# nabeelscicom/DistilCodec_nabeel

Measured on AMD Instinct MI355X. Metric: 24 kHz samples/s encode+decode at 1/8 GPU; code-index bit-exact vs CPU, higher is better.
Workload: dtype f32

## Files before the change

distilcodec_nabeel_amd/csrc/dcx_conv_common.h:

```cpp
#pragma once
#include <algorithm>
#include <type_traits>

#include "dcx_kernels.h"
#include "dcx_planes.h"

namespace dcx {

typedef float f32x16 __attribute__((ext_vector_type(16)));
typedef float f32x4 __attribute__((ext_vector_type(4)));
typedef float f32x2 __attribute__((ext_vector_type(2)));
typedef short s16x8 __attribute__((ext_vector_type(8)));
typedef short s16x4 __attribute__((ext_vector_type(4)));
typedef __bf16 bf16x8 __attribute__((ext_vector_type(8)));

constexpr int BK = 16;
constexpr int LDSK = 20;
template <bool SWZ>
struct XRow {
  static constexpr int kStride = SWZ ? 48 : 56;
  __device__ static __forceinline__ int half(int row, int h) { return SWZ ? h ^ ((row >> 3) & 1) : h; }
  __device__ static __forceinline__ int off(int row, int piece) {
    const int h = piece >= 3;
    return row * kStride + (half(row, h) * 3 + piece - 3 * h) * 8;
  }
};

__device__ __forceinline__ float silu_f(float v) { return v * __builtin_amdgcn_rcpf(1.0f + __expf(-v)); }
__device__ __forceinline__ float gelu_f(float v) { return 0.5f * v * (1.0f + erff(v * 0.70710678118654752440f)); }
__device__ __forceinline__ float gelu_bf16_f(float v) {
#ifdef DCX_GELU_ERF
  return gelu_f(v);
#endif
  const float z = fabsf(v) * 0.70710678118654752440f;
  const float t = __builtin_amdgcn_rcpf(fmaf(0.5f, z, 1.0f));
  float q = 0.17087277f;
  q = fmaf(q, t, -0.82215223f);
  q = fmaf(q, t, 1.48851587f);
  q = fmaf(q, t, -1.13520398f);
  q = fmaf(q, t, 0.27886807f);
  q = fmaf(q, t, -0.18628806f);
  q = fmaf(q, t, 0.09678418f);
  q = fmaf(q, t, 0.37409196f);
  q = fmaf(q, t, 1.00002368f);
  const float c = t * __expf(fmaf(t, q, fmaf(-z, z, -1.26551223f)));
  const float e = v >= 0.0f ? 1.0f - c : c - 1.0f;
  return 0.5f * v * (1.0f + e);
}

__device__ __forceinline__ f32x2 gelu_bf16_f2(f32x2 v) {
#ifdef DCX_GELU_SCALAR
  return f32x2{gelu_bf16_f(v[0]), gelu_bf16_f(v[1])};
#endif
  const f32x2 z = __builtin_elementwise_abs(v) * 0.70710678118654752440f;
  const f32x2 d = __builtin_elementwise_fma(f32x2{0.5f, 0.5f}, z, f32x2{1.0f, 1.0f});
  const f32x2 t = {__builtin_amdgcn_rcpf(d[0]), __builtin_amdgcn_rcpf(d[1])};
  auto fm = [&](f32x2 q, float c) { return __builtin_elementwise_fma(q, t, f32x2{c, c}); };
  f32x2 q = {0.17087277f, 0.17087277f};
  q = fm(q, -0.82215223f);
  q = fm(q, 1.48851587f);
  q = fm(q, -1.13520398f);
  q = fm(q, 0.27886807f);
  q = fm(q, -0.18628806f);
  q = fm(q, 0.09678418f);
  q = fm(q, 0.37409196f);
  q = fm(q, 1.00002368f);
  const f32x2 arg = __builtin_elementwise_fma(t, q, __builtin_elementwise_fma(-z, z, f32x2{-1.26551223f, -1.26551223f}));
  const f32x2 c = t * f32x2{__expf(arg[0]), __expf(arg[1])};
  const f32x2 e = {v[0] >= 0.0f ? 1.0f - c[0] : c[0] - 1.0f, v[1] >= 0.0f ? 1.0f - c[1] : c[1] - 1.0f};
  return 0.5f * v * (1.0f + e);
}

__device__ __forceinline__ int xcd_remap(int bid, int nwg) {
  const int xcd = bid & 7, q = nwg >> 3, r = nwg & 7;
  return (xcd < r ? xcd * (q + 1) : r * (q + 1) + (xcd - r) * q) + (bid >> 3);
}

__device__ __forceinline__ void flat_tile(int tpc, int batch, int& wg, int& b, int& ph) {
  const int t = xcd_remap(blockIdx.x, gridDim.x);
  const int per_ph = tpc * batch;
  ph = t / per_ph;
  const int r = t - ph * per_ph;
  b = r / tpc;
  wg = r - b * tpc;
}

__device__ __forceinline__ void ksplit_slice(const ConvParams& p, int b, int& clip, int& c0, int& nchunks) {
  clip = b;
  c0 = 0;
  nchunks = p.Cin / BK;
  if (p.ksplit > 1) {
    const int clips = p.batch / p.ksplit, sl = b / clips;
    clip = b - sl * clips;
    const int nunits = nchunks / p.kunit, base = nunits / p.ksplit, extra = nunits % p.ksplit;
    c0 = (sl * base + min(sl, extra)) * p.kunit;
    nchunks = (base + (sl < extra ? 1 : 0)) * p.kunit;
  }
}

static __device__ __attribute__((used, aligned(16))) float g_zero_row[32] = {0.f};

#if defined(DCX_CLOCK_DIAG) || defined(DCX_SEG_DIAG) || defined(DCX_TILE_DIAG)
#define DCX_DIAG 1
constexpr int kTileDiagMax = 16384;
[[maybe_unused]] static __device__ unsigned long long g_clock_diag[3], g_seg_diag[13], g_seg_diag8[49];
[[maybe_unused]] static __device__ unsigned long long g_tile_diag[kTileDiagMax * 6];
[[maybe_unused]] static __device__ unsigned int g_tile_cnt;
enum DiagSet : int { DIAG_CLOCK, DIAG_SEG, DIAG_SEG8, DIAG_TILES };
static int diag_read(int set, unsigned long long* out, int n, int reset) {
  if (set == DIAG_TILES) {
    unsigned int cnt = 0;
    if (hipMemcpyFromSymbol(&cnt, HIP_SYMBOL(g_tile_cnt), sizeof cnt) != hipSuccess) return -1;
    cnt = std::min(cnt, (unsigned)std::max(0, std::min(n, kTileDiagMax)));
    if (cnt && hipMemcpyFromSymbol(out, HIP_SYMBOL(g_tile_diag), sizeof(unsigned long long) * 6 * cnt) != hipSuccess) return -1;
    const unsigned int z = 0;
    if (reset && hipMemcpyToSymbol(HIP_SYMBOL(g_tile_cnt), &z, sizeof z) != hipSuccess) return -1;
    return (int)cnt;
  }
  const void* sym = set == DIAG_CLOCK ? (const void*)g_clock_diag : set == DIAG_SEG ? (const void*)g_seg_diag : (const void*)g_seg_diag8;
  unsigned long long v[49] = {};
  if (n > 49 || hipMemcpyFromSymbol(v, sym, sizeof(unsigned long long) * n) != hipSuccess) return -1;
  for (int i = 0; i < n; ++i) out[i] += v[i];
  const unsigned long long z[49] = {};
  if (reset && hipMemcpyToSymbol(sym, z, sizeof(unsigned long long) * n) != hipSuccess) return -1;
  return 0;
}
#define DCX_DIAG_FILE(tag) \
  int diag_##tag(int set, unsigned long long* out, int n, int reset) { return diag_read(set, out, n, reset); }
#else
#define DCX_DIAG_FILE(tag)
#endif
#ifdef DCX_SEG_DIAG
#define DCX_SEGT(v) const unsigned long long v = __builtin_amdgcn_s_memtime()
#else
#define DCX_SEGT(v)
#endif
#ifdef DCX_TILE_DIAG
#define DCX_TILET(v) const unsigned long long v = __builtin_amdgcn_s_memrealtime()
#else
#define DCX_TILET(v)
#endif

struct EpiPre {
  int osh;
  float acur;
  bool track;
};
template <int RROW>
__device__ __forceinline__ EpiPre epi_range_pre(const ConvParams& p, const ConvParams& pr, int b) {
  EpiPre e{0, 0.f, false};
  const bool h2o = (p.y6 && p.y_layout == LAYOUT_H2) || (p.y6s && p.ys_layout != LAYOUT_PLANES);
  const bool h2row = (RROW & 2) && h2o && pr.yb.rowwise;
  if (h2o && !h2row) {
    const float bnd = range_bound(pr.yb, b);
    e.osh = __builtin_amdgcn_readfirstlane(h2_shift(bnd));
    if (threadIdx.x == 0) {
      if (pr.y_ash) pr.y_ash[b] = e.osh;
      if (pr.rflag && !(bnd <= 3.0e38f)) atomicOr(pr.rflag, RANGE_NONFINITE);
    }
  }
  const bool track = pr.y_amax != nullptr;
  e.track = track;
  e.acur = track && !h2row ? __builtin_bit_cast(float, __builtin_amdgcn_readfirstlane(
                                                           __builtin_bit_cast(int, range_cur(pr.y_amax, b))))
                           : 0.f;
  return e;
}

struct EpiGeneric {
  static constexpr bool fixed = false;
};
template <int EPI, int MEAN, bool Y, bool Y2, bool Y6H, bool Y6SH, bool TRACK, bool ROWWISE = false>
struct EpiForm {
  static constexpr bool fixed = true;
  static constexpr int epi = EPI, mean = MEAN;
  static constexpr bool y = Y, y2 = Y2, y6h = Y6H, y6sh = Y6SH, track = TRACK, rowwise = ROWWISE;
};
template <typename F>
inline bool epi_form_is(const ConvParams& p) {
  const bool h2o = F::y6h || F::y6sh;
  return p.epi == F::epi && p.mean_mode == F::mean && !p.round_bf16 && (p.y != nullptr) == F::y &&
         (p.y2 != nullptr) == F::y2 && (p.y6 != nullptr) == F::y6h && (p.y6s != nullptr) == F::y6sh &&
         (!p.y6 || p.y_layout == LAYOUT_H2) && (!p.y6s || p.ys_layout == LAYOUT_H2) && (p.y_amax != nullptr) == F::track &&
         (h2o ? (p.yb.rowwise != 0) == F::rowwise : true) && (F::epi != EPI_GELU || p.w6 != nullptr) &&
         (F::mean == MEAN_NONE || p.macc != nullptr);
}

template <int BM, int BN, int WM, int WN, int LDS_FLOATS, int NT, int RROW, bool RAG, typename F, typename AccT>
__device__ __forceinline__ void epilogue_form(const ConvParams& p, const ConvParams& pr, AccT& acc, int q0, int co0, int b,
                                              int ph, float* smem, const EpiPre& pre) {
  constexpr int WR = BM / WM, WC = BN / WN;
  static_assert(sizeof(acc[0][0]) == 16 && sizeof(acc) == WR * WC * 4 / 64, "16 x 16 accumulator blocks");
  constexpr int LDSW = BN + 4;
  constexpr int RPP = (BM * LDSW <= LDS_FLOATS) ? BM
                      : (BM / 2 * LDSW <= LDS_FLOATS) ? BM / 2
                      : (BM / 4 * LDSW <= LDS_FLOATS) ? BM / 4 : WR;
  static_assert(RPP % WR == 0 && RPP * LDSW <= LDS_FLOATS, "epilogue pass does not fit LDS");
  const int tid = threadIdx.x, lane = tid & 63, wave = tid >> 6;
  const int wm = wave / WN, wn = wave % WN;
  const long long ob = (long long)b * p.y_bstride;
  constexpr bool RIN = RROW & 1, ROUT = RROW & 2;
  constexpr bool h2o = F::y6h || F::y6sh, h2row = ROUT && h2o && F::rowwise;
  constexpr bool need_r = F::epi == EPI_GAMMA_RES || F::epi == EPI_RES;
  constexpr bool need_m = F::mean == MEAN_MID || F::mean == MEAN_LAST;
  static_assert(!((F::mean == MEAN_FIRST || F::mean == MEAN_MID) && (F::y || F::y2 || h2o || F::track)), "mean form");
  unsigned short* const y6 = F::y6h ? p.y6 + ob * 2 : nullptr;
  unsigned short* const y6s = F::y6sh ? p.y6s + ob * 2 : nullptr;
  const float osc = __builtin_bit_cast(
      float, __builtin_amdgcn_readfirstlane(__builtin_bit_cast(int, __builtin_ldexpf(1.0f, h2o && !h2row ? pre.osh : 0))));
  float vmax = 0.f;
  const int lq_live = RAG ? clip_rows(pr.clip_len, pr.len_mul, b, p.Lq) : p.Lq;
  constexpr int G = 8, NH = 2;
  static_assert(NT % (BN / G) == 0, "each thread keeps one channel group");
  const int cg = (tid % (BN / G)) * G, trow = tid / (BN / G), co = co0 + cg;
  const int hsw = (lane >> 3) & 1;
  f32x4 bias4[NH], gamma4[NH];
#pragma unroll
  for (int h = 0; h < NH; ++h) {
    bias4[h] = p.bias ? *reinterpret_cast<const f32x4*>(p.bias + co + 4 * h) : f32x4{0.f, 0.f, 0.f, 0.f};
    gamma4[h] = F::epi == EPI_GAMMA_RES ? *reinterpret_cast<const f32x4*>(p.gamma + co + 4 * h) : f32x4{0.f, 0.f, 0.f, 0.f};
  }
  constexpr int RSTEP = NT / (BN / G), ROWS_T = RPP / RSTEP;
  static_assert(RPP % RSTEP == 0, "epilogue rows per thread");
  constexpr auto div_cap = [](int n, int cap) {
    int d = n < cap ? n : cap;
    while (n % d) --d;
    return d;
  };
  constexpr int IB = div_cap(ROWS_T, need_r || need_m ? 4 / NH : 8 / NH);
  auto row_bound = [&](int q) { return fmaf(pr.yb.g[0], fmaxf(pr.yb.m[0][(long long)b * p.Lq + q], pr.yb.f[0]), pr.yb.c); };

  auto pass = [&](int r0, auto fullt) {
    constexpr bool FULL = decltype(fullt)::value;
    f32x4 r[IB][NH], m[IB][NH];
    float rin[RIN ? IB : 1], rbnd[h2row ? IB : 1];
    auto load = [&](int rb) {
#pragma unroll
      for (int k = 0; k < IB; ++k) {
        const int qq = q0 + r0 + trow + (rb + k) * RSTEP;
        const int q = FULL ? qq : min(qq, p.Lq - 1);
        const long long o = ob + ((long long)q * p.out_mul + ph) * p.ldy + co;
#pragma unroll
        for (int h = 0; h < NH; ++h) {
          if constexpr (need_r) r[k][h] = *reinterpret_cast<const f32x4*>(p.res + o + 4 * h);
          if constexpr (need_m) m[k][h] = *reinterpret_cast<const f32x4*>(p.macc + o + 4 * h);
        }
        if constexpr (RIN) rin[k] = pr.x_ash_row ? __builtin_ldexpf(1.0f, -pr.x_ash_row[(long long)b * p.Lin + q]) : 1.0f;
        if constexpr (h2row) rbnd[k] = row_bound(q);
      }
    };
    load(0);
    __syncthreads();
    if (wm * WR >= r0 && wm * WR < r0 + RPP) {
#pragma unroll
      for (int i = 0; i < WR / 16; ++i)
#pragma unroll
        for (int j = 0; j < WC / 16; ++j)
#pragma unroll
          for (int e = 0; e < 4; ++e) {
            const int row = wm * WR + i * 16 + 4 * (lane >> 4) + e - r0;
            smem[row * LDSW + wn * WC + j * 16 + (lane & 15)] = acc[i][j][e];
          }
    }
    __syncthreads();
#pragma unroll
    for (int rb = 0; rb < ROWS_T; rb += IB) {
      f32x4 x[IB][NH];
      float rsc[IB];
#pragma unroll
      for (int k = 0; k < IB; ++k) {
        const int rl = trow + (rb + k) * RSTEP;
        const int q = q0 + r0 + rl;
        const bool dead = RAG && q >= lq_live;
        const float rin_ = RIN ? rin[RIN ? k : 0] : 1.0f;
        const f32x4 u = *reinterpret_cast<const f32x4*>(smem + rl * LDSW + cg + 4 * hsw);
        const f32x4 v = *reinterpret_cast<const f32x4*>(smem + rl * LDSW + cg + 4 * (1 - hsw));
        x[k][0] = (hsw ? v : u) * rin_ + bias4[0];
        x[k][1] = (hsw ? u : v) * rin_ + bias4[1];
#pragma unroll
        for (int h = 0; h < NH; ++h) {
          if constexpr (F::epi == EPI_GELU) {
#pragma unroll
            for (int e = 0; e < 4; e += 2) {
              const f32x2 g = gelu_bf16_f2(f32x2{x[k][h][e], x[k][h][e + 1]});
              x[k][h][e] = g[0];
              x[k][h][e + 1] = g[1];
            }
          } else if constexpr (F::epi == EPI_GAMMA_RES) {
            x[k][h] = r[k][h] + gamma4[h] * x[k][h];
          } else if constexpr (F::epi == EPI_RES) {
            x[k][h] = r[k][h] + x[k][h];
          } else {
            static_assert(F::epi == EPI_BIAS, "epilogue form");
          }
          if (dead) x[k][h] = f32x4{0.f, 0.f, 0.f, 0.f};
          if constexpr (F::mean == MEAN_MID) x[k][h] = dead ? x[k][h] : m[k][h] + x[k][h];
          if constexpr (F::mean == MEAN_LAST) x[k][h] = dead ? x[k][h] : (m[k][h] + x[k][h]) / 3.0f;
        }
        rsc[k] = osc;
        if constexpr (h2row) rsc[k] = rbnd[k];
      }
      if (rb + IB < ROWS_T) load(rb + IB);
#pragma unroll
      for (int k = 0; k < IB; ++k) {
        const int q = q0 + r0 + trow + (rb + k) * RSTEP;
        if (!FULL && q >= p.Lq) continue;
        const long long orow = (long long)q * p.out_mul + ph;
        const long long o = ob + orow * p.ldy + co;
        if constexpr (F::mean == MEAN_FIRST || F::mean == MEAN_MID) {
#pragma unroll
          for (int h = 0; h < NH; ++h) *reinterpret_cast<f32x4*>(p.macc + o + 4 * h) = x[k][h];
          continue;
        }
        float sc = rsc[k];
        if constexpr (h2row) {
          const float bnd = rsc[k];
          const int sh = h2_shift(bnd);
          sc = __builtin_ldexpf(1.0f, sh);
          if (cg == 0 && pr.y_ash) pr.y_ash[(long long)b * p.Lq + q] = sh;
          if (pr.rflag && !(bnd <= 3.0e38f)) atomicOr(pr.rflag, RANGE_NONFINITE);
        }
        if constexpr (F::track) {
          const float ts = h2row ? sc : 1.0f;
#pragma unroll
          for (int h = 0; h < NH; ++h)
#pragma unroll
            for (int e = 0; e < 4; ++e) vmax = fmaxf(vmax, fabsf(x[k][h][e]) * ts);
        }
        if constexpr (F::y) {
#pragma unroll
          for (int h = 0; h < NH; ++h) *reinterpret_cast<f32x4*>(p.y + o + 4 * h) = x[k][h];
        }
        float xv[8];
#pragma unroll
        for (int e = 0; e < 8; ++e) xv[e] = x[k][e >> 2][e & 3];
        if constexpr (F::y6h) store_h2_8<false>(y6, orow, p.Cout, co, xv, sc);
        if constexpr (F::y2 || F::y6sh) {
          float sv[8];
#pragma unroll
          for (int e = 0; e < 8; ++e) sv[e] = silu_f(xv[e]);
          if constexpr (F::y2) {
            *reinterpret_cast<f32x4*>(p.y2 + o) = f32x4{sv[0], sv[1], sv[2], sv[3]};
            *reinterpret_cast<f32x4*>(p.y2 + o + 4) = f32x4{sv[4], sv[5], sv[6], sv[7]};
          }
          if constexpr (F::y6sh) store_h2_8<false>(y6s, orow, p.Cout, co, sv, sc);
        }
      }
    }
  };
#pragma unroll 1
  for (int r0 = 0; r0 < BM; r0 += RPP) {
    if (q0 + r0 + RPP <= p.Lq) pass(r0, std::true_type{});
    else pass(r0, std::false_type{});
  }
  if constexpr (F::track)
    range_report_wg(vmax, h2row ? nullptr : pr.y_amax, b, h2row ? 65504.0f : h2o ? 65504.0f / osc : __builtin_inff(),
                    pr.rflag, pre.acur, smem, NT);
}

template <int BM, int BN, int WM, int WN, int LDS_FLOATS, int NT, int RROW = 2, bool RAG = true, typename F = EpiGeneric,
          typename AccT>
__device__ __forceinline__ void epilogue_lds(const ConvParams& p, const ConvParams& pr, AccT& acc, int q0, int co0,
                                             int b, int ph, float* smem, const EpiPre* pre = nullptr) {
#ifndef DCX_EPI4
  if constexpr (F::fixed) {
    epilogue_form<BM, BN, WM, WN, LDS_FLOATS, NT, RROW, RAG, F>(p, pr, acc, q0, co0, b, ph, smem, *pre);
    return;
  }
#endif
  constexpr int WR = BM / WM, WC = BN / WN;
  constexpr int TM = WR / 32, TN = WC / 32;
  constexpr bool M16 = sizeof(acc[0][0]) == 16;
  static_assert(sizeof(acc) == WR * WC * 4 / 64, "accumulator tile");
  constexpr int LDSW = BN + 4;
  constexpr int RPP = (BM * LDSW <= LDS_FLOATS) ? BM
                      : (BM / 2 * LDSW <= LDS_FLOATS) ? BM / 2
                      : (BM / 4 * LDSW <= LDS_FLOATS) ? BM / 4 : WR;
  static_assert(RPP % WR == 0 && RPP * LDSW <= LDS_FLOATS, "epilogue pass does not fit LDS");
  const int tid = threadIdx.x, lane = tid & 63, wave = tid >> 6;
  const int wm = wave / WN, wn = wave % WN;
  const int lrow = lane & 31, rhalf = 4 * (lane >> 5);
  const long long ob = (long long)b * p.y_bstride;
  unsigned short* y6 = p.y6 ? p.y6 + ob * layout_u16(p.y_layout) : nullptr;
  unsigned short* y6s = p.y6s ? p.y6s + ob * (p.ys_layout != LAYOUT_PLANES ? 2 : 3) : nullptr;
  const bool h2o = (y6 && p.y_layout == LAYOUT_H2) || (y6s && p.ys_layout != LAYOUT_PLANES);
  constexpr bool RIN = RROW & 1, ROUT = RROW & 2;
  const bool h2row = ROUT && h2o && pr.yb.rowwise;
  int osh = 0;
  if (pre) {
    osh = pre->osh;
  } else if (h2o && !h2row) {
    const float bnd = range_bound(pr.yb, b);
    osh = __builtin_amdgcn_readfirstlane(h2_shift(bnd));
    if (tid == 0) {
      if (pr.y_ash) pr.y_ash[b] = osh;
      if (pr.rflag && !(bnd <= 3.0e38f)) atomicOr(pr.rflag, RANGE_NONFINITE);
    }
  }
  const float osc =
      __builtin_bit_cast(float, __builtin_amdgcn_readfirstlane(__builtin_bit_cast(int, __builtin_ldexpf(1.0f, osh))));
#ifdef DCX_DIAG_NORANGE
  const bool track = false;
#else
  const bool track = pre ? pre->track : pr.y_amax != nullptr;
#endif
  const float acur = pre ? pre->acur : track && !h2row ? range_cur(pr.y_amax, b) : 0.f;
  float vmax = 0.f;
  const int lq_live = RAG ? clip_rows(pr.clip_len, pr.len_mul, b, p.Lq) : p.Lq;
#ifdef DCX_EPI4
  constexpr int G = 4;
#else
  constexpr int G = 8;
#endif
  constexpr int NH = G / 4;
  static_assert(NT % (BN / G) == 0, "each thread keeps one channel group");
  const int cg = (tid % (BN / G)) * G, trow = tid / (BN / G), co = co0 + cg;
  const int hsw = G == 8 ? (lane >> 3) & 1 : 0;
  f32x4 bias4[NH], gamma4[NH];
#pragma unroll
  for (int h = 0; h < NH; ++h) {
    bias4[h] = p.bias ? *reinterpret_cast<const f32x4*>(p.bias + co + 4 * h) : f32x4{0.f, 0.f, 0.f, 0.f};
    gamma4[h] = p.epi == EPI_GAMMA_RES ? *reinterpret_cast<const f32x4*>(p.gamma + co + 4 * h) : f32x4{0.f, 0.f, 0.f, 0.f};
  }
#ifdef DCX_DIAG_NOEPI
  if (q0 >= 0) return;
#endif
#ifdef DCX_DIAG_DUP
  if (p.diag_skip == 2) return;
#endif
  auto stage_acc = [&](int r0) {
    __syncthreads();
    if (wm * WR >= r0 && wm * WR < r0 + RPP) {
      if constexpr (M16) {
#pragma unroll
        for (int i = 0; i < WR / 16; ++i)
#pragma unroll
          for (int j = 0; j < WC / 16; ++j)
#pragma unroll
            for (int e = 0; e < 4; ++e) {
              const int row = wm * WR + i * 16 + 4 * (lane >> 4) + e - r0;
              smem[row * LDSW + wn * WC + j * 16 + (lane & 15)] = acc[i][j][e];
            }
      } else {
#pragma unroll
        for (int i = 0; i < TM; ++i)
#pragma unroll
          for (int j = 0; j < TN; ++j)
#pragma unroll
            for (int r = 0; r < 16; ++r) {
              const int row = wm * WR + i * 32 + (r & 3) + 8 * (r >> 2) + rhalf - r0;
              smem[row * LDSW + wn * WC + j * 32 + lrow] = acc[i][j][r];
            }
      }
    }
    __syncthreads();
  };
  constexpr int RSTEP = NT / (BN / G), ROWS_T = RPP / RSTEP;
  static_assert(RPP % RSTEP == 0, "epilogue rows per thread");
  const bool need_r = p.epi == EPI_GAMMA_RES || p.epi == EPI_RES;
  const bool need_m = p.mean_mode == MEAN_MID || p.mean_mode == MEAN_LAST;
  auto batch = [&](int r0, int rb, bool stage, auto ibt) {
    constexpr int IB = decltype(ibt)::value;
    f32x4 r[IB][NH], m[IB][NH];
    auto lofs = [&](int k) {
      const int q = min(q0 + r0 + trow + (rb + k) * RSTEP, p.Lq - 1);
      return ob + ((long long)q * p.out_mul + ph) * p.ldy + co;
    };
    if (need_r) {
#pragma unroll
      for (int k = 0; k < IB; ++k)
#pragma unroll
        for (int h = 0; h < NH; ++h) r[k][h] = *reinterpret_cast<const f32x4*>(p.res + lofs(k) + 4 * h);
    }
    if (need_m) {
#pragma unroll
      for (int k = 0; k < IB; ++k)
#pragma unroll
        for (int h = 0; h < NH; ++h) m[k][h] = *reinterpret_cast<const f32x4*>(p.macc + lofs(k) + 4 * h);
    }
    auto row_bound = [&](int q) { return fmaf(pr.yb.g[0], fmaxf(pr.yb.m[0][(long long)b * p.Lq + q], pr.yb.f[0]), pr.yb.c); };
    float rin[RIN ? IB : 1], rbnd[RIN ? IB : 1];
    if constexpr (RIN) {
#pragma unroll
      for (int k = 0; k < IB; ++k) {
        const int q = min(q0 + r0 + trow + (rb + k) * RSTEP, p.Lq - 1);
        rin[k] = pr.x_ash_row ? __builtin_ldexpf(1.0f, -pr.x_ash_row[(long long)b * p.Lin + q]) : 1.0f;
        rbnd[k] = h2row ? row_bound(q) : 0.f;
      }
    }
    if (stage) stage_acc(r0);
#pragma unroll
    for (int k = 0; k < IB; ++k) {
      const int rl = trow + (rb + k) * RSTEP;
      const int q = q0 + r0 + rl;
      if (q >= p.Lq) continue;
      const long long orow = (long long)q * p.out_mul + ph;
      const long long o = ob + orow * p.ldy + co;
      f32x4 x[NH];
      const float rin_ = RIN ? rin[RIN ? k : 0] : 1.0f;
      if constexpr (NH == 2) {
        const f32x4 u = *reinterpret_cast<const f32x4*>(smem + rl * LDSW + cg + 4 * hsw);
        const f32x4 v = *reinterpret_cast<const f32x4*>(smem + rl * LDSW + cg + 4 * (1 - hsw));
        x[0] = (hsw ? v : u) * rin_ + bias4[0];
        x[1] = (hsw ? u : v) * rin_ + bias4[1];
      } else {
        x[0] = *reinterpret_cast<const f32x4*>(smem + rl * LDSW + cg) * rin_ + bias4[0];
      }
#pragma unroll
      for (int h = 0; h < NH; ++h) {
        if (p.round_bf16) x[h] = round_bf16x4(x[h]);
        switch (p.epi) {
          case EPI_GELU:
            if (p.w6) {
#ifndef DCX_EPI_NOGELU
#pragma unroll
              for (int e = 0; e < 4; e += 2) {
                const f32x2 g = gelu_bf16_f2(f32x2{x[h][e], x[h][e + 1]});
                x[h][e] = g[0];
                x[h][e + 1] = g[1];
              }
#endif
              if (p.round_bf16 && (p.y || y6s || p.y2 || p.y_layout != LAYOUT_BF16)) x[h] = round_bf16x4(x[h]);
            } else {
#pragma unroll
              for (int e = 0; e < 4; ++e) x[h][e] = gelu_f(x[h][e]);
            }
            break;
          case EPI_GAMMA_RES: x[h] = r[k][h] + gamma4[h] * x[h]; break;
          case EPI_RES:
            x[h] = r[k][h] + x[h];
            if (p.round_bf16) x[h] = round_bf16x4(x[h]);
            break;
          case EPI_LOGCLAMP:
#pragma unroll
            for (int e = 0; e < 4; ++e) x[h][e] = logf(fmaxf(x[h][e], 1e-5f));
            break;
          default: break;
        }
        if (RAG && q >= lq_live) x[h] = f32x4{0.f, 0.f, 0.f, 0.f};
      }
#ifdef DCX_EPI_NOSTORE
      if (x[0][0] != -0x1.234p-100f) continue;
#endif
#ifdef DCX_DIAG_DUP
      if (p.diag_skip == 1 && x[0][0] != -0x1.234p-100f) continue;
#endif
      if (p.mean_mode == MEAN_FIRST) {
#pragma unroll
        for (int h = 0; h < NH; ++h) *reinterpret_cast<f32x4*>(p.macc + o + 4 * h) = x[h];
        continue;
      } else if (p.mean_mode == MEAN_MID) {
#pragma unroll
        for (int h = 0; h < NH; ++h) *reinterpret_cast<f32x4*>(p.macc + o + 4 * h) = RAG && q >= lq_live ? x[h] : m[k][h] + x[h];
        continue;
      } else if (p.mean_mode == MEAN_LAST) {
#pragma unroll
        for (int h = 0; h < NH; ++h) {
          x[h] = RAG && q >= lq_live ? x[h] : (m[k][h] + x[h]) / 3.0f;
          if (p.round_bf16) x[h] = round_bf16x4(x[h]);
        }
      }
      float rsc = osc;
      if (h2row) {
        const long long grow = (long long)b * p.Lq + q;
        const float bnd = RIN ? rbnd[RIN ? k : 0] : row_bound(q);
        const int sh = h2_shift(bnd);
        rsc = __builtin_ldexpf(1.0f, sh);
        if (cg == 0 && pr.y_ash) pr.y_ash[grow] = sh;
        if (pr.rflag && !(bnd <= 3.0e38f)) atomicOr(pr.rflag, RANGE_NONFINITE);
      }
      if (track) {
        const float ts = h2row ? rsc : 1.0f;
#pragma unroll
        for (int h = 0; h < NH; ++h)
#pragma unroll
          for (int e = 0; e < 4; ++e) vmax = fmaxf(vmax, fabsf(x[h][e]) * ts);
      }
      if (p.y) {
#pragma unroll
        for (int h = 0; h < NH; ++h) *reinterpret_cast<f32x4*>(p.y + o + 4 * h) = x[h];
      }
      if constexpr (G == 8) {
        float xv[8];
#pragma unroll
        for (int e = 0; e < 8; ++e) xv[e] = x[e >> 2][e & 3];
        if (y6) {
          if (p.y_layout == LAYOUT_BF16) store_bf16x8(y6, orow, p.Cout, co, xv);
          else if ((int)p.y_layout == 2) store_hm8(y6, orow, p.Cout, co, xv);
          else if (p.y_layout == LAYOUT_H2) store_h2_8<false>(y6, orow, p.Cout, co, xv, rsc);
          else store_planes8(y6, orow, p.Cout, co, xv);
        }
        if (p.y2 || y6s) {
          float sv[8];
#pragma unroll
          for (int e = 0; e < 8; ++e) sv[e] = p.round_bf16 ? bf16_val(bf16_bits(silu_f(xv[e]))) : silu_f(xv[e]);
          if (p.y2) {
            *reinterpret_cast<f32x4*>(p.y2 + o) = f32x4{sv[0], sv[1], sv[2], sv[3]};
            *reinterpret_cast<f32x4*>(p.y2 + o + 4) = f32x4{sv[4], sv[5], sv[6], sv[7]};
          }
          if (y6s) {
            if (p.ys_layout != LAYOUT_PLANES) store_h2_8<false>(y6s, orow, p.Cout, co, sv, rsc);
            else store_planes8(y6s, orow, p.Cout, co, sv);
          }
        }
      } else {
        if (y6) {
          if (p.y_layout == LAYOUT_BF16) store_bf16x4(y6, orow, p.Cout, co, x[0][0], x[0][1], x[0][2], x[0][3]);
          else if ((int)p.y_layout == 2) store_hm4(y6, orow, p.Cout, co, x[0][0], x[0][1], x[0][2], x[0][3]);
          else if (p.y_layout == LAYOUT_H2) store_h2_4<false>(y6, orow, p.Cout, co, x[0][0], x[0][1], x[0][2], x[0][3], rsc);
          else store_planes4(y6, orow, p.Cout, co, x[0][0], x[0][1], x[0][2], x[0][3]);
        }
        if (p.y2 || y6s) {
          f32x4 sv;
#pragma unroll
          for (int e = 0; e < 4; ++e) sv[e] = p.round_bf16 ? bf16_val(bf16_bits(silu_f(x[0][e]))) : silu_f(x[0][e]);
          if (p.y2) *reinterpret_cast<f32x4*>(p.y2 + o) = sv;
          if (y6s) {
            if (p.ys_layout != LAYOUT_PLANES) store_h2_4<false>(y6s, orow, p.Cout, co, sv[0], sv[1], sv[2], sv[3], rsc);
            else store_planes4(y6s, orow, p.Cout, co, sv[0], sv[1], sv[2], sv[3]);
          }
        }
      }
    }
  };
  constexpr int IBF0 = 8 / NH, IBM0 = 4 / NH;
  constexpr auto div_cap = [](int n, int cap) {
    int d = n < cap ? n : cap;
    while (n % d) --d;
    return d;
  };
  constexpr int IBF = div_cap(ROWS_T, IBF0), IBM = div_cap(ROWS_T, IBM0);
  static_assert(ROWS_T % IBF == 0 && ROWS_T % IBM == 0, "epilogue batches");
#pragma unroll 1
  for (int r0 = 0; r0 < BM; r0 += RPP) {
    if (need_m) {
#pragma unroll
      for (int rb = 0; rb < ROWS_T; rb += IBM) batch(r0, rb, rb == 0, std::integral_constant<int, IBM>{});
    } else {
#pragma unroll
      for (int rb = 0; rb < ROWS_T; rb += IBF) batch(r0, rb, rb == 0, std::integral_constant<int, IBF>{});
    }
  }
  if (track)
    range_report_wg(vmax, h2row ? nullptr : pr.y_amax, b, h2row ? 65504.0f : h2o ? 65504.0f / osc : __builtin_inff(),
                    pr.rflag, acur, smem, NT);
}

__device__ __forceinline__ bool tile_dead(const ConvParams& p, const ConvParams& pr, int b, int q0) {
  return pr.clip_len != nullptr && q0 >= clip_rows(pr.clip_len, pr.len_mul, b, p.Lq);
}
template <int BM, int BN, int NT>
__device__ __forceinline__ void epilogue_dead(const ConvParams& p, const ConvParams& pr, int q0, int co0, int b, int ph) {
  const long long ob = (long long)b * p.y_bstride;
  unsigned short* y6 = p.y6 ? p.y6 + ob * layout_u16(p.y_layout) : nullptr;
  unsigned short* y6s = p.y6s ? p.y6s + ob * (p.ys_layout != LAYOUT_PLANES ? 2 : 3) : nullptr;
  const bool h2o = (y6 && p.y_layout == LAYOUT_H2) || (y6s && p.ys_layout != LAYOUT_PLANES);
  if (h2o && threadIdx.x == 0) {
    const float bnd = range_bound(pr.yb, b);
    if (pr.y_ash) pr.y_ash[b] = h2_shift(bnd);
    if (pr.rflag && !(bnd <= 3.0e38f)) atomicOr(pr.rflag, RANGE_NONFINITE);
  }
  const f32x4 z4 = {0.f, 0.f, 0.f, 0.f};
  const float z8[8] = {0.f, 0.f, 0.f, 0.f, 0.f, 0.f, 0.f, 0.f};
  constexpr int CG = BN / 8;
  for (int i = threadIdx.x; i < BM * CG; i += NT) {
    const int q = q0 + i / CG, co = co0 + (i % CG) * 8;
    if (q >= p.Lq) break;
    const long long orow = (long long)q * p.out_mul + ph;
    const long long o = ob + orow * p.ldy + co;
    if (p.mean_mode == MEAN_FIRST || p.mean_mode == MEAN_MID) {
      *reinterpret_cast<f32x4*>(p.macc + o) = z4;
      *reinterpret_cast<f32x4*>(p.macc + o + 4) = z4;
      continue;
    }
    if (p.y) {
      *reinterpret_cast<f32x4*>(p.y + o) = z4;
      *reinterpret_cast<f32x4*>(p.y + o + 4) = z4;
    }
    if (y6) {
      if (p.y_layout == LAYOUT_BF16) store_bf16x8(y6, orow, p.Cout, co, z8);
      else if (p.y_layout == LAYOUT_H2) store_h2_8<false>(y6, orow, p.Cout, co, z8, 1.0f);
      else store_planes8(y6, orow, p.Cout, co, z8);
    }
    if (p.y2) {
      *reinterpret_cast<f32x4*>(p.y2 + o) = z4;
      *reinterpret_cast<f32x4*>(p.y2 + o + 4) = z4;
    }
    if (y6s) {
      if (p.ys_layout != LAYOUT_PLANES) store_h2_8<false>(y6s, orow, p.Cout, co, z8, 1.0f);
      else store_planes8(y6s, orow, p.Cout, co, z8);
    }
  }
}

typedef __attribute__((address_space(3))) void* lds_ptr_t;

__device__ __forceinline__ void dma16(__amdgpu_buffer_rsrc_t r, unsigned short* lds, int voff, int soff) {
  __builtin_amdgcn_raw_ptr_buffer_load_lds(r, (lds_ptr_t)lds, 16, voff, soff, 0, 0);
}
__device__ __forceinline__ void seg_barrier() { asm volatile("s_waitcnt lgkmcnt(0)\n\ts_barrier" ::: "memory"); }
__device__ __forceinline__ void wait_dma(int n) {
#define DCX_W(k) \
  case k: asm volatile("s_waitcnt vmcnt(" #k ")" ::: "memory"); break;
  switch (n) {
    DCX_W(1) DCX_W(2) DCX_W(3) DCX_W(4) DCX_W(5) DCX_W(6) DCX_W(7) DCX_W(8) DCX_W(9) DCX_W(10) DCX_W(11)
    DCX_W(12) DCX_W(13) DCX_W(14) DCX_W(15) DCX_W(16) DCX_W(17) DCX_W(18) DCX_W(19) DCX_W(20) DCX_W(21) DCX_W(22)
    DCX_W(23)
    default: asm volatile("s_waitcnt vmcnt(0)" ::: "memory");
  }
#undef DCX_W
}

}
```

distilcodec_nabeel_amd/csrc/dcx_planes.h:

```cpp
#pragma once
#include <hip/hip_runtime.h>

namespace dcx {

typedef short s16x4p __attribute__((ext_vector_type(4)));

__device__ __forceinline__ unsigned short bf16_bits(float x) { return __builtin_bit_cast(unsigned short, (__bf16)x); }
__device__ __forceinline__ float bf16_val(unsigned short b) { return __uint_as_float((unsigned)b << 16); }

typedef float f32x4p __attribute__((ext_vector_type(4)));
__device__ __forceinline__ f32x4p round_bf16x4(f32x4p v) {
#pragma unroll
  for (int e = 0; e < 4; ++e) v[e] = bf16_val(bf16_bits(v[e]));
  return v;
}

__device__ __forceinline__ void split3(float x, unsigned short& h, unsigned short& m, unsigned short& l) {
  h = bf16_bits(x);
  const float r1 = x - bf16_val(h);
  m = bf16_bits(r1);
  const float r2 = r1 - bf16_val(m);
  l = bf16_bits(r2);
}

__device__ __forceinline__ long long plane_off(long long row, int C, int c) {
  return row * (long long)C * 3 + (c >> 3) * 24 + (c & 7);
}

__device__ __forceinline__ void store_planes1(unsigned short* base, long long row, int C, int c, float v) {
  unsigned short h, m, l;
  split3(v, h, m, l);
  unsigned short* d = base + plane_off(row, C, c);
  d[0] = h;
  d[8] = m;
  d[16] = l;
}

__device__ __forceinline__ void store_planes4(unsigned short* base, long long row, int C, int c, float a, float b,
                                              float cc, float d) {
  s16x4p hv, mv, lv;
  const float v[4] = {a, b, cc, d};
#pragma unroll
  for (int e = 0; e < 4; ++e) {
    unsigned short h, m, l;
    split3(v[e], h, m, l);
    hv[e] = (short)h;
    mv[e] = (short)m;
    lv[e] = (short)l;
  }
  unsigned short* dst = base + plane_off(row, C, c);
  *reinterpret_cast<s16x4p*>(dst) = hv;
  *reinterpret_cast<s16x4p*>(dst + 8) = mv;
  *reinterpret_cast<s16x4p*>(dst + 16) = lv;
}

__device__ __forceinline__ void store_bf16x4(unsigned short* base, long long row, int C, int c, float a, float b,
                                             float cc, float d) {
  s16x4p hv;
  hv[0] = (short)bf16_bits(a);
  hv[1] = (short)bf16_bits(b);
  hv[2] = (short)bf16_bits(cc);
  hv[3] = (short)bf16_bits(d);
  *reinterpret_cast<s16x4p*>(base + row * (long long)C + c) = hv;
}

__device__ __forceinline__ void store_hm4(unsigned short* base, long long row, int C, int c, float a, float b,
                                          float cc, float d) {
  s16x4p hv, mv;
  const float v[4] = {a, b, cc, d};
#pragma unroll
  for (int e = 0; e < 4; ++e) {
    unsigned short h, m, l;
    split3(v[e], h, m, l);
    hv[e] = (short)h;
    mv[e] = (short)m;
  }
  unsigned short* dst = base + row * (long long)C * 2 + (c >> 5) * 64 + ((c >> 3) & 3) * 16 + (c & 7);
  *reinterpret_cast<s16x4p*>(dst) = hv;
  *reinterpret_cast<s16x4p*>(dst + 8) = mv;
}

typedef short s16x8p __attribute__((ext_vector_type(8)));
__device__ __forceinline__ void store_planes8(unsigned short* base, long long row, int C, int c, const float (&v)[8]) {
  s16x8p hv, mv, lv;
#pragma unroll
  for (int e = 0; e < 8; ++e) {
    unsigned short h, m, l;
    split3(v[e], h, m, l);
    hv[e] = (short)h;
    mv[e] = (short)m;
    lv[e] = (short)l;
  }
  unsigned short* dst = base + plane_off(row, C, c);
  *reinterpret_cast<s16x8p*>(dst) = hv;
  *reinterpret_cast<s16x8p*>(dst + 8) = mv;
  *reinterpret_cast<s16x8p*>(dst + 16) = lv;
}

__device__ __forceinline__ void store_bf16x8(unsigned short* base, long long row, int C, int c, const float (&v)[8]) {
  s16x8p hv;
#pragma unroll
  for (int e = 0; e < 8; ++e) hv[e] = (short)bf16_bits(v[e]);
  *reinterpret_cast<s16x8p*>(base + row * (long long)C + c) = hv;
}

__device__ __forceinline__ void store_hm8(unsigned short* base, long long row, int C, int c, const float (&v)[8]) {
  s16x8p hv, mv;
#pragma unroll
  for (int e = 0; e < 8; ++e) {
    unsigned short h, m, l;
    split3(v[e], h, m, l);
    hv[e] = (short)h;
    mv[e] = (short)m;
  }
  unsigned short* dst = base + row * (long long)C * 2 + (c >> 5) * 64 + ((c >> 3) & 3) * 16;
  *reinterpret_cast<s16x8p*>(dst) = hv;
  *reinterpret_cast<s16x8p*>(dst + 8) = mv;
}

template <bool SAT = true>
__device__ __forceinline__ void split2h(float x, unsigned short& h, unsigned short& l) {
  const float xs = !SAT ? x : fabsf(x) > 65504.f ? copysignf(65504.f, x) : x;
  const _Float16 hh = (_Float16)xs;
  h = __builtin_bit_cast(unsigned short, hh);
  l = __builtin_bit_cast(unsigned short, (_Float16)(xs - (float)hh));
}
__device__ __forceinline__ void split2h_nc(float x, unsigned short& h, unsigned short& l) { split2h<false>(x, h, l); }
template <bool SAT = true>
__device__ __forceinline__ void store_h2_4(unsigned short* base, long long row, int C, int c, float a, float b,
                                           float cc, float d, float sc = 1.0f) {
  s16x4p hv, lv;
  const float v[4] = {a * sc, b * sc, cc * sc, d * sc};
#pragma unroll
  for (int e = 0; e < 4; ++e) {
    unsigned short h, l;
    split2h<SAT>(v[e], h, l);
    hv[e] = (short)h;
    lv[e] = (short)l;
  }
  unsigned short* dst = base + row * (long long)C * 2 + (c >> 5) * 64 + ((c >> 3) & 3) * 16 + (c & 7);
  *reinterpret_cast<s16x4p*>(dst) = hv;
  *reinterpret_cast<s16x4p*>(dst + 8) = lv;
}
template <bool SAT = true>
__device__ __forceinline__ void store_h2_8(unsigned short* base, long long row, int C, int c, const float (&v)[8],
                                           float sc = 1.0f) {
  s16x8p hv, lv;
#pragma unroll
  for (int e = 0; e < 8; ++e) {
    unsigned short h, l;
    split2h<SAT>(v[e] * sc, h, l);
    hv[e] = (short)h;
    lv[e] = (short)l;
  }
  unsigned short* dst = base + row * (long long)C * 2 + (c >> 5) * 64 + ((c >> 3) & 3) * 16;
  *reinterpret_cast<s16x8p*>(dst) = hv;
  *reinterpret_cast<s16x8p*>(dst + 8) = lv;
}

}
```

Before: 52.86 million.

## Use 4-channel-per-thread epilogue lines with DPP-exchanged fp16 plane stores

For RROW==0 epilogues (except one residual BN=256 ragged case), each thread now handles 4 channels instead of 8. It reads one contiguous f32x4 from LDS rather than two swapped halves. The hi/lo fp16 plane writes pair neighbouring lanes via a DPP swap, so each lane writes a full 16-byte line. The goal is fewer LDS bank conflicts and less register pressure in the epilogue, at the cost of more rows per thread and cross-lane shuffles.

```diff
diff --git a/distilcodec_nabeel_amd/csrc/dcx_conv_common.h b/distilcodec_nabeel_amd/csrc/dcx_conv_common.h
--- a/distilcodec_nabeel_amd/csrc/dcx_conv_common.h
+++ b/distilcodec_nabeel_amd/csrc/dcx_conv_common.h
@@ -210,8 +210,9 @@
       float, __builtin_amdgcn_readfirstlane(__builtin_bit_cast(int, __builtin_ldexpf(1.0f, h2o && !h2row ? pre.osh : 0))));
   float vmax = 0.f;
   const int lq_live = RAG ? clip_rows(pr.clip_len, pr.len_mul, b, p.Lq) : p.Lq;
-  constexpr int G = 8, NH = 2;
-  static_assert(NT % (BN / G) == 0, "each thread keeps one channel group");
+  constexpr bool LINES = RROW == 0 && !(RAG && BN == 256 && need_r && (F::mean == MEAN_NONE || F::mean == MEAN_LAST));
+  constexpr int G = LINES ? kEpiG : 8, NH = G / 4;
+  static_assert(NT % (BN / G) == 0 && LDSW == epi_ldsw(BN), "each thread keeps one channel group");
   const int cg = (tid % (BN / G)) * G, trow = tid / (BN / G), co = co0 + cg;
   const int hsw = (lane >> 3) & 1;
   f32x4 bias4[NH], gamma4[NH];
@@ -221,7 +222,7 @@
     gamma4[h] = F::epi == EPI_GAMMA_RES ? *reinterpret_cast<const f32x4*>(p.gamma + co + 4 * h) : f32x4{0.f, 0.f, 0.f, 0.f};
   }
   constexpr int RSTEP = NT / (BN / G), ROWS_T = RPP / RSTEP;
-  static_assert(RPP % RSTEP == 0, "epilogue rows per thread");
+  static_assert(RPP % RSTEP == 0 && (!LINES || RSTEP == epi_rstep(NT, BN)), "epilogue rows per thread");
   constexpr auto div_cap = [](int n, int cap) {
     int d = n < cap ? n : cap;
     while (n % d) --d;
@@ -273,10 +274,14 @@
         const int q = q0 + r0 + rl;
         const bool dead = RAG && q >= lq_live;
         const float rin_ = RIN ? rin[RIN ? k : 0] : 1.0f;
-        const f32x4 u = *reinterpret_cast<const f32x4*>(smem + rl * LDSW + cg + 4 * hsw);
-        const f32x4 v = *reinterpret_cast<const f32x4*>(smem + rl * LDSW + cg + 4 * (1 - hsw));
-        x[k][0] = (hsw ? v : u) * rin_ + bias4[0];
-        x[k][1] = (hsw ? u : v) * rin_ + bias4[1];
+        if constexpr (LINES) {
+          x[k][0] = *reinterpret_cast<const f32x4*>(smem + epi_lds_float(rl, tid, BN)) * rin_ + bias4[0];
+        } else {
+          const f32x4 u = *reinterpret_cast<const f32x4*>(smem + rl * LDSW + cg + 4 * hsw);
+          const f32x4 v = *reinterpret_cast<const f32x4*>(smem + rl * LDSW + cg + 4 * (1 - hsw));
+          x[k][0] = (hsw ? v : u) * rin_ + bias4[0];
+          x[k][NH - 1] = (hsw ? u : v) * rin_ + bias4[NH - 1];
+        }
 #pragma unroll
         for (int h = 0; h < NH; ++h) {
           if constexpr (F::epi == EPI_GELU) {
@@ -331,19 +336,30 @@
 #pragma unroll
           for (int h = 0; h < NH; ++h) *reinterpret_cast<f32x4*>(p.y + o + 4 * h) = x[k][h];
         }
-        float xv[8];
-#pragma unroll
-        for (int e = 0; e < 8; ++e) xv[e] = x[k][e >> 2][e & 3];
-        if constexpr (F::y6h) store_h2_8<false>(y6, orow, p.Cout, co, xv, sc);
-        if constexpr (F::y2 || F::y6sh) {
-          float sv[8];
-#pragma unroll
-          for (int e = 0; e < 8; ++e) sv[e] = silu_f(xv[e]);
-          if constexpr (F::y2) {
-            *reinterpret_cast<f32x4*>(p.y2 + o) = f32x4{sv[0], sv[1], sv[2], sv[3]};
-            *reinterpret_cast<f32x4*>(p.y2 + o + 4) = f32x4{sv[4], sv[5], sv[6], sv[7]};
+        if constexpr (LINES) {
+          if constexpr (F::y6h) store_h2_pair<false>(y6, orow, p.Cout, co, x[k][0], sc);
+          if constexpr (F::y2 || F::y6sh) {
+            f32x4 sv;
+#pragma unroll
+            for (int e = 0; e < 4; ++e) sv[e] = silu_f(x[k][0][e]);
+            if constexpr (F::y2) *reinterpret_cast<f32x4*>(p.y2 + o) = sv;
+            if constexpr (F::y6sh) store_h2_pair<false>(y6s, orow, p.Cout, co, sv, sc);
           }
-          if constexpr (F::y6sh) store_h2_8<false>(y6s, orow, p.Cout, co, sv, sc);
+        } else {
+          float xv[8];
+#pragma unroll
+          for (int e = 0; e < 8; ++e) xv[e] = x[k][e >> 2][e & 3];
+          if constexpr (F::y6h) store_h2_8<false>(y6, orow, p.Cout, co, xv, sc);
+          if constexpr (F::y2 || F::y6sh) {
+            float sv[8];
+#pragma unroll
+            for (int e = 0; e < 8; ++e) sv[e] = silu_f(xv[e]);
+            if constexpr (F::y2) {
+              *reinterpret_cast<f32x4*>(p.y2 + o) = f32x4{sv[0], sv[1], sv[2], sv[3]};
+              *reinterpret_cast<f32x4*>(p.y2 + o + 4) = f32x4{sv[4], sv[5], sv[6], sv[7]};
+            }
+            if constexpr (F::y6sh) store_h2_8<false>(y6s, orow, p.Cout, co, sv, sc);
+          }
         }
       }
     }
diff --git a/distilcodec_nabeel_amd/csrc/dcx_epi_lines.h b/distilcodec_nabeel_amd/csrc/dcx_epi_lines.h
--- /dev/null
+++ b/distilcodec_nabeel_amd/csrc/dcx_epi_lines.h
@@ -0,0 +1,23 @@
+#pragma once
+
+#if defined(__HIPCC__) || defined(__CUDACC__)
+#define DCX_EPI_HD __host__ __device__
+#else
+#define DCX_EPI_HD
+#endif
+
+namespace dcx {
+
+constexpr int kEpiG = 4;
+
+DCX_EPI_HD constexpr int epi_chan(int tid, int BN) { return (tid % (BN / kEpiG)) * kEpiG; }
+DCX_EPI_HD constexpr int epi_row0(int tid, int BN) { return tid / (BN / kEpiG); }
+DCX_EPI_HD constexpr int epi_rstep(int NT, int BN) { return NT / (BN / kEpiG); }
+DCX_EPI_HD constexpr int epi_ldsw(int BN) { return BN + 4; }
+DCX_EPI_HD constexpr int epi_lds_float(int rl, int tid, int BN) { return rl * epi_ldsw(BN) + epi_chan(tid, BN); }
+DCX_EPI_HD constexpr int epi_f32_off(int co0, int tid, int BN) { return co0 + epi_chan(tid, BN); }
+DCX_EPI_HD constexpr int epi_h2_unit(int c) { return c >> 3; }
+DCX_EPI_HD constexpr bool epi_h2_odd(int c) { return (c & 4) != 0; }
+DCX_EPI_HD constexpr int epi_h2_off(int c) { return epi_h2_unit(c) * 16 + (epi_h2_odd(c) ? 8 : 0); }
+
+}
diff --git a/distilcodec_nabeel_amd/csrc/dcx_planes.h b/distilcodec_nabeel_amd/csrc/dcx_planes.h
--- a/distilcodec_nabeel_amd/csrc/dcx_planes.h
+++ b/distilcodec_nabeel_amd/csrc/dcx_planes.h
@@ -1,5 +1,7 @@
 #pragma once
 #include <hip/hip_runtime.h>
+
+#include "dcx_epi_lines.h"
 
 namespace dcx {
 
@@ -157,5 +159,19 @@
   *reinterpret_cast<s16x8p*>(dst) = hv;
   *reinterpret_cast<s16x8p*>(dst + 8) = lv;
 }
+template <bool SAT = true>
+__device__ __forceinline__ void store_h2_pair(unsigned short* base, long long row, int C, int c4, const f32x4p& v,
+                                              float sc = 1.0f) {
+  unsigned short h[4], l[4];
+#pragma unroll
+  for (int e = 0; e < 4; ++e) split2h<SAT>(v[e] * sc, h[e], l[e]);
+  const int h0 = h[0] | (h[1] << 16), h1 = h[2] | (h[3] << 16), l0 = l[0] | (l[1] << 16), l1 = l[2] | (l[3] << 16);
+  const bool odd = epi_h2_odd(c4);
+  const int g0 = __builtin_amdgcn_mov_dpp(odd ? h0 : l0, 0xB1, 0xF, 0xF, true);
+  const int g1 = __builtin_amdgcn_mov_dpp(odd ? h1 : l1, 0xB1, 0xF, 0xF, true);
+  typedef int i32x4p __attribute__((ext_vector_type(4)));
+  const i32x4p o = odd ? i32x4p{g0, g1, l0, l1} : i32x4p{h0, h1, g0, g1};
+  *reinterpret_cast<i32x4p*>(base + row * (long long)C * 2 + epi_h2_off(c4)) = o;
+}
 
 }
```

Measured after the change: 53.43 million, median of 6. +1.1%, better.
